# qianduoduolr/FGVC

Measured on AMD Instinct MI355X. Metric: frames/sec + ms/corr-volume, 480p 8-frame clip, 1/2/4/8 MI355X, higher is better.
Workload: dtype f16 + fp6 (e2m3) MFMA operands, f32 accumulate; top-k near-ties re-scored in f64 from f32 features

## Files before the change

### fgvc_amd/csrc/capi.hip

```cpp
#include <stdarg.h>
#include <string.h>

#include "common.hpp"

namespace fgvc {

static thread_local char g_err[512] = "";

void set_error(const char* fmt, ...) {
  va_list ap;
  va_start(ap, fmt);
  vsnprintf(g_err, sizeof(g_err), fmt, ap);
  va_end(ap);
}

int pair_topk_launch(const float*, const float*, const int32_t*, int, int, int, int, int, int, int, int, int, int,
                     const uint8_t*, int32_t*, float*, hipStream_t);
int merge_topk_launch(const int32_t*, const float*, const int32_t*, int, int, int, int, int, float, int, int32_t*,
                      float*, float*, hipStream_t);
int normalize_launch(const float*, float*, int, int, int, int, int, hipStream_t);
int propagate_launch(const float*, const int32_t*, int, const int32_t*, const float*, int, int, int, int, int, int,
                     int, float*, hipStream_t);
int bn_act_launch(const float*, const float*, const float*, const float*, const float*, const float*, float, int, float*,
                  int, int, int, hipStream_t);
int gaussian_launch(const float*, int, int, int, int, float, float*, hipStream_t);
int softargmax_launch(const float*, int, int, int, int, int, int, const float*, float, double*, float*, hipStream_t);
int softargmax_bands();
int corr_volume_f32_launch(const float*, const float*, int, int, int, float, float*, hipStream_t);
int split_bf16_launch(const float*, uint16_t*, long long, int, hipStream_t);
int corr_volume_bf16_launch(const uint16_t*, const uint16_t*, int, int, int, float, float*, int, hipStream_t);
int local_merge_launch(const int32_t*, const float*, int, int, int, int, int, float, int32_t*, float*, float*,
                       hipStream_t);
int local_merge_plan_launch(const int32_t*, const float*, const int32_t*, int, int, int, int, int, int, int, float, int32_t*, float*,
                            float*, hipStream_t);
int topk_coord_launch(const int32_t*, const float*, int, int, int, int, int, float*, hipStream_t);
int topk_coord_rows_launch(const int32_t*, const float*, int, int, int, int, int, int, float*, hipStream_t);
int cycle_chase_launch(const float*, const float*, const float*, int, int, int, int, int, float*, float*, hipStream_t);
int flow_from_lists_launch(const int32_t*, const float*, int, int, int, int, int, int, int, int, int, int, int, float*, uint8_t*, hipStream_t);
int flow_consistency_launch(const float*, const float*, int, int, int, int, float, float*, float*, hipStream_t);
int warp_launch(const float*, const float*, int, int, int, int, int, int, float*, hipStream_t);
int frames_rgb8_to_lab_launch(const uint8_t*, int, int, int, long long, long long, long long, long long, int, int, int, int, int, int, float*,
                              hipStream_t);
int jf_counts_launch(const uint8_t*, const uint8_t*, int, int, int, int, int, int64_t*, hipStream_t);
int jf_tile_rows();
int render_frames_launch(const uint8_t*, long long, long long, uint8_t*, long long, long long, int, int, int, const uint8_t*, long long, long long,
                         const uint8_t*, int, int, const double*, long long, long long, const uint8_t*, long long, long long, const uint8_t*, int,
                         int, const double*, hipStream_t);
void render_tile(int*, int*);
int c2f_refine_launch(const int32_t*, const float*, const float*, const float*, int, int, int, int, int, int, int,
                      int, float, int, float*, int32_t*, float*, hipStream_t);

int conv_split_launch(const uint16_t*, const uint16_t*, const float*, const float*, uint16_t*, float*, int, int, int, int, int,
                      int, int, int, int, int, int, int, int, int*, hipStream_t, unsigned char* y_bank = nullptr, int bank_normalize = 1, const uint16_t* x2 = nullptr,
                      const uint16_t* w2 = nullptr, int Cin2 = 0, int bank_row_bytes = 1024);
int conv_s2_launch(const uint16_t*, const uint16_t*, const float*, uint16_t*, float*, int, int, int, int, int, int, int, int, int,
                   int, int, int, int, int*, const uint16_t*, const float*, float*, int, hipStream_t);
int conv64_launch(const uint16_t*, const uint16_t*, const float*, const float*, const uint16_t*, uint16_t*, float*, int, int, int, int, int, int,
                  int, int, int, int, int*, hipStream_t);
int stem7_launch(const float*, const uint16_t*, const float*, uint16_t*, float*, int, int, int, int, int, int, int, int, int, int, int*,
                 hipStream_t);
int nchw_to_split_nhwc_launch(const float*, uint16_t*, float*, int, int, int, int, int, int, hipStream_t);
int normalize_nhwc_launch(const float*, float*, uint16_t*, int, int, int, int, int, int, hipStream_t);
int nhwc_to_split_launch(float*, uint16_t*, int, int, int, int, int, int, int, hipStream_t);

void set_conv_cot_cap(int);
void set_conv_narrow(int);
void set_conv64_variant(int);
int conv64_probe_read(long long*);
void set_conv_debug(int);
void set_corr6_skew(int);
void set_corr6_sdma(int);
void set_pair_debug(int);
void set_readout_prune(int);
void set_conv_s2_debug(int);
int split_f16x2_launch(const float*, uint16_t*, long long, int, hipStream_t);
int split_f16f6p_launch(const float*, unsigned char*, long long, int, hipStream_t);
int pair_topk_v7_launch(const uint16_t*, const uint16_t*, const int32_t*, int, int, int, int, int, int, int, int, int, const int32_t*, int,
                        int32_t*, float*, int, hipStream_t);
int pair_topk_v5_launch(const uint16_t*, const uint16_t*, const int32_t*, int, int, int, int, int, int, int, int, int, int, const int32_t*,
                        int, int32_t*, float*, hipStream_t);
// ... 41 lines not shown
               "fgvc_set_option: %s = %d switches a profiling ablation on (bits %d: results would be wrong); this library is built without them -- "
               "use libfgvc_hip_ablations.so (FGVC_HIP_LIB)", name, value, ablation_bits(name, value));
#endif
  if (strcmp(name, "corr_debug") == 0) {
    set_corr_debug(value);
    return FGVC_OK;
  }
  if (strcmp(name, "corr8_debug") == 0) {
    set_corr8_debug(value);
    return FGVC_OK;
  }
  if (strcmp(name, "corr6_debug") == 0) {
    set_corr6_debug(value);
    return FGVC_OK;
  }
  if (strcmp(name, "pair_debug") == 0) {
    set_pair_debug(value);
    return FGVC_OK;
  }
  if (strcmp(name, "corr6_sdma") == 0) {
    set_corr6_sdma(value);
    return FGVC_OK;
  }
  if (strcmp(name, "corr6_skew") == 0) {
    set_corr6_skew(value);
    return FGVC_OK;
  }
  if (strcmp(name, "conv_debug") == 0) {
    set_conv_debug(value);
    return FGVC_OK;
  }
  if (strcmp(name, "conv64_variant") == 0) {
    set_conv64_variant(value);
    return FGVC_OK;
  }
  if (strcmp(name, "conv_narrow") == 0) {
    set_conv_narrow(value);
    return FGVC_OK;
  }
  if (strcmp(name, "conv_cot_cap") == 0) {
    FGVC_REQUIRE(value == 0 || value == 64 || value == 128, FGVC_ERR_INVALID_ARG, "fgvc_set_option: conv_cot_cap must be 0, 64 or 128");
    set_conv_cot_cap(value);
    return FGVC_OK;
  }
  if (strcmp(name, "pair_f16_debug") == 0) {
    set_pair_v5_debug(value);
    return FGVC_OK;
  }
  if (strcmp(name, "conv_s2_debug") == 0) {
    set_conv_s2_debug(value);
    return FGVC_OK;
  }
  if (strcmp(name, "readout_prune") == 0) {
    set_readout_prune(value != 0);
    return FGVC_OK;
  }
  set_error("fgvc_set_option: unknown option '%s'", name);
  return FGVC_ERR_INVALID_ARG;
}

int fgvc_r2max_for_radius(float radius) {
  if (!(radius > 0.f)) return -1;
  long long d2 = (long long)ceil((double)radius * (double)radius) + 2;
  if (d2 > FGVC_NO_LIMIT) return FGVC_NO_LIMIT;
  while (d2 >= 0 && !(sqrtf((float)d2) < radius)) --d2;
  return (int)d2;
}

int fgvc_normalize_chw_to_hwc_f32(const float* in, float* out, int n, int C, int HW, int normalize, int c_out,
                                  void* stream) {
  FGVC_REQUIRE(in && out, FGVC_ERR_INVALID_ARG, "fgvc_normalize_chw_to_hwc_f32: null pointer");
  FGVC_REQUIRE(n >= 0 && C > 0 && HW > 0, FGVC_ERR_INVALID_ARG, "fgvc_normalize_chw_to_hwc_f32: bad shape n=%d C=%d HW=%d", n, C, HW);
  FGVC_REQUIRE(C <= 1024, FGVC_ERR_UNSUPPORTED, "fgvc_normalize_chw_to_hwc_f32: C=%d > 1024 (LDS tile)", C);
  FGVC_REQUIRE(n <= 65535, FGVC_ERR_UNSUPPORTED, "fgvc_normalize_chw_to_hwc_f32: n=%d > 65535 frames per call", n);
  FGVC_REQUIRE(c_out >= C, FGVC_ERR_INVALID_ARG, "fgvc_normalize_chw_to_hwc_f32: c_out=%d < C=%d", c_out, C);
  if (n == 0) return FGVC_OK;
  return normalize_launch(in, out, n, C, HW, normalize, c_out, (hipStream_t)stream);
}

int fgvc_pair_topk_f32(const float* qfeat, const float* kfeat, const int32_t* pairs, int n_pairs, int C, int Hq,
                       int Wq, int Hk, int Wk, int r2max, int ry, int rx, int topk, const uint8_t* dense_mask,
                       int32_t* idx_out, float* score_out, void* stream) {
  FGVC_REQUIRE(qfeat && kfeat && pairs && idx_out && score_out, FGVC_ERR_INVALID_ARG, "fgvc_pair_topk_f32: null pointer");
  FGVC_REQUIRE(aligned16(qfeat) && aligned16(kfeat) && aligned16(pairs), FGVC_ERR_INVALID_ARG,
               "fgvc_pair_topk_f32: qfeat/kfeat/pairs must be 16-byte aligned");
  FGVC_REQUIRE(Hq > 0 && Wq > 0 && Hk > 0 && Wk > 0 && n_pairs >= 0, FGVC_ERR_INVALID_ARG,
               "fgvc_pair_topk_f32: bad shape Hq=%d Wq=%d Hk=%d Wk=%d n_pairs=%d", Hq, Wq, Hk, Wk, n_pairs);
  FGVC_REQUIRE(topk >= 1 && topk <= 16, FGVC_ERR_UNSUPPORTED, "fgvc_pair_topk_f32: topk=%d outside 1..16", topk);
  FGVC_REQUIRE(r2max >= 0 && ry >= 0 && rx >= 0, FGVC_ERR_INVALID_ARG, "fgvc_pair_topk_f32: negative mask parameter");
  FGVC_REQUIRE(n_pairs <= 65535, FGVC_ERR_UNSUPPORTED, "fgvc_pair_topk_f32: n_pairs=%d > 65535 per call", n_pairs);
  const bool any_limit = r2max < FGVC_NO_LIMIT || ry < FGVC_NO_LIMIT || rx < FGVC_NO_LIMIT;
  FGVC_REQUIRE(!any_limit || (Hq == Hk && Wq == Wk), FGVC_ERR_INVALID_ARG,
               "fgvc_pair_topk_f32: a spatial mask needs equal query/key grids (local_attention.py:331)");
  FGVC_REQUIRE((long long)Hk * Wk < (1ll << 30) && (long long)Hq * Wq < (1ll << 30), FGVC_ERR_UNSUPPORTED,
               "fgvc_pair_topk_f32: grid too large");
  if (n_pairs == 0) return FGVC_OK;
  FGVC_REQUIRE(dense_mask == nullptr || !any_limit, FGVC_ERR_INVALID_ARG,
               "fgvc_pair_topk_f32: give either the analytic predicate or a dense mask, not both");
  return pair_topk_launch(qfeat, kfeat, pairs, n_pairs, C, Hq, Wq, Hk, Wk, r2max, ry, rx, topk, dense_mask, idx_out,
                          score_out, (hipStream_t)stream);
}

int fgvc_split_f16x2(const float* feat, uint16_t* h_l, int64_t n_pixels, int C, void* stream) {
  FGVC_REQUIRE(feat && h_l, FGVC_ERR_INVALID_ARG, "fgvc_split_f16x2: null pointer");
  FGVC_REQUIRE(n_pixels >= 0 && C > 0 && C % 4 == 0, FGVC_ERR_INVALID_ARG, "fgvc_split_f16x2: C must be a multiple of 4");
  FGVC_REQUIRE(aligned16(feat) && aligned16(h_l), FGVC_ERR_INVALID_ARG, "fgvc_split_f16x2: 16-byte alignment required");
  if (n_pixels == 0) return FGVC_OK;
// ... 687 lines not shown
  FGVC_REQUIRE(x && out, FGVC_ERR_INVALID_ARG, "fgvc_nhwc_to_split_f32: null pointer");
  FGVC_REQUIRE(N >= 0 && C > 0 && C % 32 == 0 && H > 0 && W > 0, FGVC_ERR_INVALID_ARG,
               "fgvc_nhwc_to_split_f32: bad shape (C must be a multiple of 32)");
  FGVC_REQUIRE(conv_pad_ok(H, W, Hp, Wp), FGVC_ERR_INVALID_ARG, "fgvc_nhwc_to_split_f32: padded size %dx%d too small for %dx%d", Hp, Wp, H, W);
  FGVC_REQUIRE(aligned16(x) && aligned16(out), FGVC_ERR_INVALID_ARG, "fgvc_nhwc_to_split_f32: 16-byte alignment required");
  FGVC_REQUIRE((long long)N * H * W * C / 4 < (1ll << 31) * 256, FGVC_ERR_UNSUPPORTED, "fgvc_nhwc_to_split_f32: tensor too large");
  if (N == 0) return FGVC_OK;
  return nhwc_to_split_launch(x, out, N, C, H, W, Hp, Wp, relu, (hipStream_t)stream);
}

static int normalize_split_common(const char* what, const float* in, float* out_f32, uint16_t* out_split, int N, int C, int H, int W,
                                  int normalize, int fmt, void* stream) {
  FGVC_REQUIRE(in && (out_f32 || out_split), FGVC_ERR_INVALID_ARG, "%s: null pointer", what);
  FGVC_REQUIRE(N >= 0 && C > 0 && C % 4 == 0 && H > 0 && W > 0, FGVC_ERR_INVALID_ARG, "%s: bad shape", what);
  FGVC_REQUIRE(aligned16(in) && aligned16(out_f32) && aligned16(out_split), FGVC_ERR_INVALID_ARG, "%s: 16-byte alignment required", what);
  if (N == 0) return FGVC_OK;
  return normalize_nhwc_launch(in, out_f32, out_split, N, C, H, W, normalize, fmt, (hipStream_t)stream);
}

int fgvc_normalize_split_nhwc_f32(const float* in, float* out_f32, uint16_t* out_split, int N, int C, int H, int W, int normalize,
                                  void* stream) {
  return normalize_split_common("fgvc_normalize_split_nhwc_f32", in, out_f32, out_split, N, C, H, W, normalize, 0, stream);
}

int fgvc_normalize_split_f16x2_nhwc_f32(const float* in, float* out_f32, uint16_t* out_split, int N, int C, int H, int W,
                                        int normalize, void* stream) {
  return normalize_split_common("fgvc_normalize_split_f16x2_nhwc_f32", in, out_f32, out_split, N, C, H, W, normalize, 1, stream);
}

int fgvc_normalize_split_f16f6p_nhwc_f32(const float* in, uint8_t* rows, int N, int C, int H, int W, int normalize, void* stream) {
  FGVC_REQUIRE(C == 256, FGVC_ERR_UNSUPPORTED, "fgvc_normalize_split_f16f6p_nhwc_f32: C=%d unsupported (256 only)", C);
  return normalize_split_common("fgvc_normalize_split_f16f6p_nhwc_f32", in, nullptr, reinterpret_cast<uint16_t*>(rows), N, C, H, W, normalize, 2, stream);
}

int fgvc_normalize_split_f16f6x_nhwc_f32(const float* in, uint8_t* rows, int N, int C, int H, int W, int normalize, void* stream) {
  FGVC_REQUIRE(C == 256, FGVC_ERR_UNSUPPORTED, "fgvc_normalize_split_f16f6x_nhwc_f32: C=%d unsupported (256 only)", C);
  return normalize_split_common("fgvc_normalize_split_f16f6x_nhwc_f32", in, nullptr, reinterpret_cast<uint16_t*>(rows), N, C, H, W, normalize, 3, stream);
}

int fgvc_normalize_nhwc_f32(const float* in, float* out, int N, int C, int H, int W, int normalize, void* stream) {
  FGVC_REQUIRE(in && out, FGVC_ERR_INVALID_ARG, "fgvc_normalize_nhwc_f32: null pointer");
  return fgvc_normalize_split_nhwc_f32(in, out, nullptr, N, C, H, W, normalize, stream);
}

int fgvc_gaussian_labels_f32(const float* points, int P, int Hf, int Wf, int stride, float sigma, float* out,
                             void* stream) {
  FGVC_REQUIRE(points && out, FGVC_ERR_INVALID_ARG, "fgvc_gaussian_labels_f32: null pointer");
  FGVC_REQUIRE(P > 0 && Hf > 0 && Wf > 0 && stride >= 1 && sigma > 0.f, FGVC_ERR_INVALID_ARG, "fgvc_gaussian_labels_f32: bad shape");
  return gaussian_launch(points, P, Hf, Wf, stride, sigma, out, (hipStream_t)stream);
}

size_t fgvc_softargmax_workspace_bytes(int n_frames, int P) {
  if (n_frames < 0 || P < 0) return 0;
  return (size_t)n_frames * P * (softargmax_bands() * (2 * 5 + 1) + 1) * sizeof(float);
}

int fgvc_softargmax_top5_f32(const float* labels, int n_frames, int Hf, int Wf, int P, int h, int w,
                             const float* gauss_points, float sigma, double* coords, void* workspace, void* stream) {
  FGVC_REQUIRE(labels && coords, FGVC_ERR_INVALID_ARG, "fgvc_softargmax_top5_f32: null pointer");
  FGVC_REQUIRE(n_frames >= 0 && Hf > 0 && Wf > 0 && P > 0 && h > 0 && w > 0, FGVC_ERR_INVALID_ARG, "fgvc_softargmax_top5_f32: bad shape");
  FGVC_REQUIRE((long long)h * w < (1ll << 31) && h * w >= 5, FGVC_ERR_UNSUPPORTED, "fgvc_softargmax_top5_f32: h*w out of range");
  FGVC_REQUIRE(n_frames <= 65535 && sigma > 0.f, FGVC_ERR_INVALID_ARG, "fgvc_softargmax_top5_f32: bad n_frames/sigma");
  FGVC_REQUIRE(workspace != nullptr || n_frames == 0, FGVC_ERR_INVALID_ARG,
               "fgvc_softargmax_top5_f32: workspace of fgvc_softargmax_workspace_bytes() bytes required");
  FGVC_REQUIRE(P <= 65535, FGVC_ERR_UNSUPPORTED, "fgvc_softargmax_top5_f32: P > 65535");
  if (n_frames == 0) return FGVC_OK;
  return softargmax_launch(labels, n_frames, Hf, Wf, P, h, w, gauss_points, sigma, coords,
                           static_cast<float*>(workspace), (hipStream_t)stream);
}

}
```

### fgvc_amd/csrc/post.hip

```cpp
#include "common.hpp"

namespace fgvc {

__global__ __launch_bounds__(256) void normalize_chw_to_hwc_kernel(const float* __restrict__ in,
                                                                     float* __restrict__ out, int C, int HW,
                                                                     int normalize, int Cout) {
  extern __shared__ float tile[];
  float* part = tile + (size_t)C * 33;
  float* inv = part + 8 * 32;
  const int tid = threadIdx.x;
  const int px = tid & 31, grp = tid >> 5;
  const int p0 = blockIdx.x * 32;
  const size_t frame = blockIdx.y;
  const float* src = in + frame * (size_t)C * HW;
  float ss = 0.f;
  const int p = p0 + px;
  for (int c = grp; c < C; c += 8) {
    const float v = (p < HW) ? src[(size_t)c * HW + p] : 0.f;
    tile[c * 33 + px] = v;
    ss = fmaf(v, v, ss);
  }
  part[grp * 32 + px] = ss;
  __syncthreads();
  if (tid < 32) {
// ... 402 lines not shown
            if (slot < RO_CELLS) cells[slot] = c;
          }
        }
      }
      __syncthreads();
      const int nc = n_cells;
      if (nc > RO_CELLS) {
        if (tid == 0) need_scan[map] = 1;
        return;
      }
      for (int k = tid >> 2; k < nc; k += RO_BLOCK / 4) {
        const int c = cells[k];
        const int i = c / Wf, j = c - i * Wf;
        const int ya = first_fine_of_cell(i, sy, Hf, h), yb = (i + 1 >= Hf) ? h : first_fine_of_cell(i + 1, sy, Hf, h);
        const int xa = first_fine_of_cell(j, sx, Wf, w), xb = (j + 1 >= Wf) ? w : first_fine_of_cell(j + 1, sx, Wf, w);
        for (int y = ya + (tid & 3); y < yb; y += 4)
          for (int x = xa; x < xb; ++x) {
            const float v = fine_value(lab, Hf, Wf, P, sy, sx, y, x);
            if (v >= tau) {
              const int slot = atomicAdd(&n_cand, 1);
              if (slot < RO_CAND) { cand_v[slot] = v; cand_i[slot] = y * w + x; }
            }
          }
      }
      __syncthreads();
      if (n_cand > RO_CAND || n_cand < K) {
        if (tid == 0) need_scan[map] = 1;
        return;
      }
    }
  }
  if (map_max > 0.f) {
    const int n = n_cand;
    for (int t = tid; t < n; t += RO_BLOCK) {
      const float v = cand_v[t];
      const int id = cand_i[t];
      int rank = 0;
      for (int u = 0; u < n; ++u) {
        const float vu = cand_v[u];
        rank += (vu > v || (vu == v && cand_i[u] > id)) ? 1 : 0;
      }
      if (rank < K) {
        part_v[o * K + rank] = v;
        part_i[o * K + rank] = id;
      }
    }
  }
  if (tid == 0) {
    part_sum[o] = map_max > 0.f ? 1.f : 0.f;
    need_scan[map] = 0;
  }
}

__global__ __launch_bounds__(64) void softargmax_merge_kernel(const float* __restrict__ part_v,
                                                               const int* __restrict__ part_i,
                                                               const float* __restrict__ part_sum, int nbands, int w,
                                                               int n_maps, double* __restrict__ coords) {
  constexpr int K = RO_K;
  const int m = blockIdx.x * 64 + threadIdx.x;
  if (m >= n_maps) return;
  TopKHi<K> top;
  top.init();
  float sum = 0.f;
  for (int b = 0; b < nbands; ++b) {
    const size_t o = (size_t)m * nbands + b;
    sum += part_sum[o];
    for (int j = 0; j < K; ++j) {
      const int id = part_i[o * K + j];
      const float v = part_v[o * K + j];
      if (id >= 0 && top.accepts(v, id)) top.insert(v, id);
    }
  }
  double* o = coords + (size_t)m * 2;
  if (sum == 0.f) {
    o[0] = -1.0;
    o[1] = -1.0;
    return;
  }
  float tot = 0.f;
#pragma unroll
  for (int j = K - 1; j >= 0; --j) tot += top.v[j];
  tot += 1e-9f;
  double ax = 0.0, ay = 0.0;
#pragma unroll
  for (int j = K - 1; j >= 0; --j) {
    const float wgt = top.v[j] / tot;
    ax += (double)(top.ix[j] % w) * (double)wgt;
    ay += (double)(top.ix[j] / w) * (double)wgt;
  }
  o[0] = ax;
  o[1] = ay;
}

template <bool VEC>
__global__ __launch_bounds__(256) void bn_act_kernel(const float* __restrict__ x, const float* __restrict__ res,
                                                      const float* __restrict__ mean, const float* __restrict__ var,
                                                      const float* __restrict__ gamma, const float* __restrict__ beta,
                                                      float eps, int relu, float* __restrict__ out, int C, int HW,
                                                      long long n) {
  const long long stride = (long long)gridDim.x * 256;
  if constexpr (VEC) {
    const long long n4 = n >> 2;
    const int HW4 = HW >> 2;
    for (long long i = (long long)blockIdx.x * 256 + threadIdx.x; i < n4; i += stride) {
      const int c = (int)((i / HW4) % C);
      const float inv = 1.0f / sqrtf(var[c] + eps);
// ... 20 lines not shown
    }
  }
}

int bn_act_launch(const float* x, const float* res, const float* mean, const float* var, const float* gamma,
                  const float* beta, float eps, int relu, float* out, int N, int C, int HW, hipStream_t s) {
  const long long n = (long long)N * C * HW;
  const bool vec = (HW % 4 == 0) && ((reinterpret_cast<uintptr_t>(x) | reinterpret_cast<uintptr_t>(out) |
                                      reinterpret_cast<uintptr_t>(res)) & 15u) == 0;
  const long long work = vec ? n / 4 : n;
  const int grid = (int)((work + 255) / 256 < 256 * 16 ? (work + 255) / 256 : 256 * 16);
  if (vec)
    bn_act_kernel<true><<<grid, 256, 0, s>>>(x, res, mean, var, gamma, beta, eps, relu, out, C, HW, n);
  else
    bn_act_kernel<false><<<grid, 256, 0, s>>>(x, res, mean, var, gamma, beta, eps, relu, out, C, HW, n);
  FGVC_CHECK_LAUNCH("fgvc_bn_act_f32");
  return FGVC_OK;
}

int normalize_launch(const float* in, float* out, int n, int C, int HW, int normalize, int Cout, hipStream_t s) {
  dim3 grid(cdiv(HW, 32), n);
  const size_t lds = ((size_t)C * 33 + 8 * 32 + 32) * sizeof(float);
  if (lds > 48 * 1024) {
    hipError_t e = hipFuncSetAttribute(reinterpret_cast<const void*>(normalize_chw_to_hwc_kernel),
                                       hipFuncAttributeMaxDynamicSharedMemorySize, (int)lds);
    if (e != hipSuccess) {
      set_error("fgvc_normalize_chw_to_hwc_f32: cannot reserve %zu B of LDS: %s", lds, hipGetErrorString(e));
      return FGVC_ERR_LAUNCH;
    }
  }
  normalize_chw_to_hwc_kernel<<<grid, 256, lds, s>>>(in, out, C, HW, normalize, Cout);
  FGVC_CHECK_LAUNCH("fgvc_normalize_chw_to_hwc_f32");
  return FGVC_OK;
}

int propagate_launch(const float* labels, const int32_t* slot_frame, int T, const int32_t* idx, const float* weight,
                     int Hq, int Wq, int Hk, int Wk, int P, int topk, int window_L, float* out, hipStream_t s) {
  const long long n = (long long)Hq * Wq * P;
  propagate_kernel<<<(unsigned)((n + 255) / 256), 256, 0, s>>>(labels, slot_frame, T, idx, weight, Hq, Wq, Hk, Wk, P,
                                                               topk, window_L, out);
  FGVC_CHECK_LAUNCH("fgvc_propagate_topk_f32");
  return FGVC_OK;
}

int gaussian_launch(const float* points, int P, int Hf, int Wf, int stride, float sigma, float* out, hipStream_t s) {
  const long long n = (long long)Hf * Wf * P;
  gaussian_labels_kernel<<<(unsigned)((n + 255) / 256), 256, 0, s>>>(points, P, Hf, Wf, stride,
                                                                     2.f * sigma * sigma, out);
  FGVC_CHECK_LAUNCH("fgvc_gaussian_labels_f32");
  return FGVC_OK;
}

int softargmax_bands() { return 8; }
static int g_readout_prune = 1;
void set_readout_prune(int v) { g_readout_prune = v; }

int softargmax_launch(const float* labels, int n_frames, int Hf, int Wf, int P, int h, int w,
                      const float* gauss_points, float sigma, double* coords, float* ws, hipStream_t s) {
  const int nb = softargmax_bands();
  const size_t maps = (size_t)n_frames * P;
  float* part_v = ws;
  int* part_i = reinterpret_cast<int*>(ws + maps * nb * RO_K);
  float* part_sum = ws + 2 * maps * nb * RO_K;
  int* need_scan = reinterpret_cast<int*>(ws + maps * nb * (2 * RO_K + 1));
  if (g_readout_prune) {
    softargmax_pruned_kernel<<<dim3(P, n_frames), RO_BLOCK, 0, s>>>(labels, Hf, Wf, P, h, w, nb, gauss_points,
                                                                2.f * sigma * sigma, part_v, part_i, part_sum, need_scan);
  }
  dim3 grid(P, n_frames, nb);
  softargmax_band_kernel<<<grid, 256, 0, s>>>(labels, Hf, Wf, P, h, w, nb, gauss_points, 2.f * sigma * sigma, part_v,
                                              part_i, part_sum, g_readout_prune ? need_scan : nullptr);
  softargmax_merge_kernel<<<cdiv((int)maps, 64), 64, 0, s>>>(part_v, part_i, part_sum, nb, w, (int)maps, coords);
  FGVC_CHECK_LAUNCH("fgvc_softargmax_top5_f32");
  return FGVC_OK;
}

}
```

### fgvc_amd/ops.py

```python
from __future__ import annotations

import ctypes as C
import functools
import math
from dataclasses import dataclass
from typing import Optional, Tuple

import torch

from . import _lib
from ._lib import NO_LIMIT, PAIR_MASKED, WEIGHT_COSINE, WEIGHT_RAW, WEIGHT_SOFTMAX


@dataclass(frozen=True)
class MaskSpec:
    r2max: int = NO_LIMIT
    ry: int = NO_LIMIT
    rx: int = NO_LIMIT

    @property
    def is_none(self) -> bool:
        return self.r2max >= NO_LIMIT and self.ry >= NO_LIMIT and self.rx >= NO_LIMIT

    @staticmethod
# ... 986 lines not shown
    x = _chk(x, torch.float32, "x")
    N, H, W, C = x.shape
    shape, dt = ((N, H * W, 4 if fmt == "f16f6x" else 2, C), torch.int16) if split else ((N, H * W, C), torch.float32)
    if out is None:
        out = torch.empty(shape, device=x.device, dtype=dt)
    else:
        assert tuple(out.shape) == shape and out.dtype == dt and out.is_contiguous() and out.device == x.device
    if fmt in ("f16f6", "f16f6x"):
        assert C == 256
        _lib.call(f"fgvc_normalize_split_{fmt}p_nhwc_f32" if fmt == "f16f6" else "fgvc_normalize_split_f16f6x_nhwc_f32", _ptr(x), _ptr(out), N, C, H, W,
                  int(normalize), _stream(x))
        return out
    _lib.call("fgvc_normalize_split_f16x2_nhwc_f32" if fmt == "f16" else "fgvc_normalize_split_nhwc_f32", _ptr(x),
              _ptr(None if split else out), _ptr(out if split else None), N, C, H, W, int(normalize), _stream(x))
    return out


def unsplit_f16x2(split: torch.Tensor) -> torch.Tensor:
    v = split.view(torch.float16).float()
    return (v[..., 0, :] + v[..., 1, :]) * (1.0 / 16384.0)


def unsplit_act(split: torch.Tensor, fmt: int, scale_log2: int = 0) -> torch.Tensor:
    n5 = split.shape
    if fmt == ACT_BF16X2:
        v = split.view(torch.bfloat16).float()
        return (v[..., :32] + v[..., 32:]).reshape(*n5[:3], -1)
    b = split.contiguous().view(torch.uint8).reshape(*n5[:4], 128)
    h = b[..., :64].contiguous().view(torch.float16).float()
    if fmt == ACT_F16X2:
        l = b[..., 64:].contiguous().view(torch.float16).float()
    elif fmt == ACT_F16F6:
        l = _e2m3_decode(torch.cat([b[..., 64:80], b[..., 96:104]], dim=-1), b[..., 104])
    else:
        l = b[..., 64:96].contiguous().view(torch.float8_e4m3fn).float() * 2.0 ** -F8_BX
    return ((h + l) * 2.0 ** -scale_log2).reshape(*n5[:3], -1)


def unsplit_bf16(split: torch.Tensor) -> torch.Tensor:
    v = split.view(torch.bfloat16).float()
    return v[..., 0, :] + v[..., 1, :]


def gaussian_labels(points: torch.Tensor, Hf: int, Wf: int, stride: int, sigma: float = 6.0,
                    out: Optional[torch.Tensor] = None) -> torch.Tensor:
    points = _chk(points.to(torch.float32), torch.float32, "points")
    P = points.shape[0]
    if out is None:
        out = torch.empty((Hf * Wf, P), device=points.device, dtype=torch.float32)
    _lib.call("fgvc_gaussian_labels_f32", _ptr(points), P, Hf, Wf, stride, float(sigma), _ptr(out), _stream(points))
    return out


def softargmax_top5(labels: torch.Tensor, Hf: int, Wf: int, h: int, w: int,
                    gauss_points: Optional[torch.Tensor] = None, sigma: float = 6.0) -> torch.Tensor:
    labels = _chk(labels, torch.float32, "labels")
    n, P = labels.shape[0], labels.shape[2]
    assert labels.shape[1] == Hf * Wf
    if gauss_points is not None:
        gauss_points = _chk(gauss_points.to(torch.float32), torch.float32, "gauss_points")
        assert gauss_points.shape == (P, 2)
    coords = torch.empty((n, P, 2), device=labels.device, dtype=torch.float64)
    ws_bytes = _lib.load().fgvc_softargmax_workspace_bytes(n, P)
    ws = torch.empty((max(ws_bytes, 4) + 3) // 4, device=labels.device, dtype=torch.float32)
    _lib.call("fgvc_softargmax_top5_f32", _ptr(labels), n, Hf, Wf, P, h, w, _ptr(gauss_points), float(sigma),
              _ptr(coords), _ptr(ws), _stream(labels))
    return coords



def pil_nearest_index(n_in: int, n_out: int) -> torch.Tensor:
    a, xo, out = n_in / n_out, n_in / n_out * 0.5, []
    for _ in range(n_out):
        out.append(min(int(xo), n_in - 1))
        xo += a
    return torch.tensor(out, dtype=torch.int64)


def seg_max_label(seg_map: torch.Tensor, Hf: int, Wf: int, out: Optional[torch.Tensor] = None) -> torch.Tensor:
    seg_map = _chk(seg_map, torch.uint8, "seg_map")
    hp, wp = seg_map.shape
    if out is None:
        out = torch.empty((1,), device=seg_map.device, dtype=torch.int32)
    _lib.call("fgvc_seg_max_label_u8", _ptr(seg_map), hp, wp, Hf, Wf, _ptr(out), _stream(seg_map))
    return out


def seg_onehot_labels(seg_map: torch.Tensor, Hf: int, Wf: int, C: int, out: Optional[torch.Tensor] = None) -> torch.Tensor:
    seg_map = _chk(seg_map, torch.uint8, "seg_map")
    hp, wp = seg_map.shape
    if out is None:
        out = torch.empty((Hf * Wf, C), device=seg_map.device, dtype=torch.float32)
    else:
        assert out.is_contiguous() and out.shape == (Hf * Wf, C) and out.dtype == torch.float32
    _lib.call("fgvc_seg_onehot_labels_u8", _ptr(seg_map), hp, wp, Hf, Wf, C, _ptr(out), _stream(seg_map))
    return out


def seg_hard_onehot(labels: torch.Tensor, out: Optional[torch.Tensor] = None) -> torch.Tensor:
    labels = _chk(labels, torch.float32, "labels")
    C = labels.shape[-1]
    if out is None:
        out = torch.empty_like(labels)
    else:
        assert out.is_contiguous() and out.shape == labels.shape and out.dtype == torch.float32
    _lib.call("fgvc_seg_hard_onehot_f32", _ptr(labels), labels.numel() // C, C, _ptr(out), _stream(labels))
    return out


def seg_readout(labels: torch.Tensor, Hf: int, Wf: int, pad_shape: Tuple[int, int], pad: Tuple[int, int, int, int],
                out_shape: Tuple[int, int], norm: bool = True, out: Optional[torch.Tensor] = None) -> torch.Tensor:
    labels = _chk(labels, torch.float32, "labels")
    n, C = labels.shape[0], labels.shape[2]
    assert labels.shape[1] == Hf * Wf
    (hp, wp), (lw, uw, lh, uh), (h0, w0) = pad_shape, pad, out_shape
    if out is None:
        out = torch.empty((n, h0, w0), device=labels.device, dtype=torch.uint8)
# ... 241 lines not shown
```

Before: 2060.

## Replace softargmax prune with chunk-stats, threshold, candidate-cell multi-kernel pipeline

Adds a new default readout pruning path built from four kernels. The first gathers per-chunk max, argmax and min over coarse label cells. The second finds a top-5 threshold tau from fine windows around the peak cells. The third collects coarse cells whose 2x2 neighbourhood bound can reach tau, and the fourth scans only those cells at fine resolution. This replaces a per-map pruned kernel, aiming to cut fine-resolution work and spread the coarse scan across many more blocks. The cost is extra launches, a larger workspace, and fallback to a full scan when the candidate count overflows RO_CELLS; the old path stays available as mode 2.

```diff
diff --git a/fgvc_amd/csrc/capi.hip b/fgvc_amd/csrc/capi.hip
--- a/fgvc_amd/csrc/capi.hip
+++ b/fgvc_amd/csrc/capi.hip
@@ -26,6 +26,7 @@
 int gaussian_launch(const float*, int, int, int, int, float, float*, hipStream_t);
 int softargmax_launch(const float*, int, int, int, int, int, int, const float*, float, double*, float*, hipStream_t);
 int softargmax_bands();
+size_t softargmax_workspace_words_per_map();
 int corr_volume_f32_launch(const float*, const float*, int, int, int, float, float*, hipStream_t);
 int split_bf16_launch(const float*, uint16_t*, long long, int, hipStream_t);
 int corr_volume_bf16_launch(const uint16_t*, const uint16_t*, int, int, int, float, float*, int, hipStream_t);
@@ -173,7 +174,8 @@
     return FGVC_OK;
   }
   if (strcmp(name, "readout_prune") == 0) {
-    set_readout_prune(value != 0);
+    FGVC_REQUIRE(value >= 0 && value <= 2, FGVC_ERR_INVALID_ARG, "fgvc_set_option: readout_prune must be 0, 1 or 2");
+    set_readout_prune(value);
     return FGVC_OK;
   }
   set_error("fgvc_set_option: unknown option '%s'", name);
@@ -967,7 +969,7 @@
 
 size_t fgvc_softargmax_workspace_bytes(int n_frames, int P) {
   if (n_frames < 0 || P < 0) return 0;
-  return (size_t)n_frames * P * (softargmax_bands() * (2 * 5 + 1) + 1) * sizeof(float);
+  return (size_t)n_frames * P * softargmax_workspace_words_per_map() * sizeof(float);
 }
 
 int fgvc_softargmax_top5_f32(const float* labels, int n_frames, int Hf, int Wf, int P, int h, int w,
diff --git a/fgvc_amd/csrc/post.hip b/fgvc_amd/csrc/post.hip
--- a/fgvc_amd/csrc/post.hip
+++ b/fgvc_amd/csrc/post.hip
@@ -478,6 +478,386 @@
   }
 }
 
+constexpr int RO_CHUNKS = 64;
+constexpr int RO_MIN_CHUNK = 32;
+constexpr int RO_LT = 16;
+constexpr int RO_T = 256;
+
+__device__ __forceinline__ int block_top5(TopKHi<RO_K>& loc, float (*sh_v)[RO_T / WAVE], int (*sh_i)[RO_T / WAVE], float (&ov)[RO_K],
+                                          int (&oi)[RO_K]) {
+  constexpr int NW = RO_T / WAVE;
+  const int lane = threadIdx.x & (WAVE - 1), wv = threadIdx.x / WAVE;
+  int n = 0;
+#pragma unroll
+  for (int r = 0; r < RO_K; ++r) {
+    float bv = loc.v[0];
+    int bi = loc.ix[0];
+#pragma unroll
+    for (int off = WAVE / 2; off >= 1; off >>= 1) {
+      const float tv = __shfl_xor(bv, off, WAVE);
+      const int ti = __shfl_xor(bi, off, WAVE);
+      const bool b = tv > bv || (tv == bv && ti > bi);
+      bv = b ? tv : bv;
+      bi = b ? ti : bi;
+    }
+    if (lane == 0) { sh_v[r][wv] = bv; sh_i[r][wv] = bi; }
+    __syncthreads();
+    bv = sh_v[r][0];
+    bi = sh_i[r][0];
+#pragma unroll
+    for (int k = 1; k < NW; ++k) {
+      const float tv = sh_v[r][k];
+      const int ti = sh_i[r][k];
+      const bool b = tv > bv || (tv == bv && ti > bi);
+      bv = b ? tv : bv;
+      bi = b ? ti : bi;
+    }
+    ov[r] = bv;
+    oi[r] = bi;
+    n += bi >= 0 ? 1 : 0;
+    const bool pop = bi >= 0 && bi == loc.ix[0];
+#pragma unroll
+    for (int j = 0; j < RO_K - 1; ++j) {
+      loc.v[j] = pop ? loc.v[j + 1] : loc.v[j];
+      loc.ix[j] = pop ? loc.ix[j + 1] : loc.ix[j];
+    }
+    loc.v[RO_K - 1] = pop ? -INFINITY : loc.v[RO_K - 1];
+    loc.ix[RO_K - 1] = pop ? -1 : loc.ix[RO_K - 1];
+  }
+  return n;
+}
+
+template <bool VEC>
+__device__ __forceinline__ void load_labels(const float* __restrict__ px, int np, float (&v)[RO_LT]) {
+  if constexpr (VEC) {
+#pragma unroll
+    for (int q = 0; q < RO_LT / 4; ++q) {
+      f32x4 t = {0.f, 0.f, 0.f, 0.f};
+      if (4 * q < np) t = reinterpret_cast<const f32x4*>(px)[q];
+      v[4 * q] = t.x; v[4 * q + 1] = t.y; v[4 * q + 2] = t.z; v[4 * q + 3] = t.w;
+    }
+  } else {
+#pragma unroll
+    for (int j = 0; j < RO_LT; ++j) v[j] = j < np ? px[j] : 0.f;
+  }
+}
+
+template <bool VEC>
+__global__ __launch_bounds__(RO_T) void softargmax_stats_kernel(const float* __restrict__ labels, int n_coarse, int P, int chunk_len,
+                                                                int skip_frame0, float* __restrict__ stats) {
+  constexpr int NW = RO_T / WAVE;
+  __shared__ float sh_mx[NW][RO_LT];
+  __shared__ int sh_am[NW][RO_LT];
+  __shared__ float sh_mn[NW][RO_LT];
+  const int tid = threadIdx.x;
+  const int chunk = blockIdx.x, f = blockIdx.y, p0 = blockIdx.z * RO_LT;
+  if (skip_frame0 && f == 0) return;
+  const int np = imin(RO_LT, P - p0);
+  const float* lab = labels + (size_t)f * n_coarse * P + p0;
+  const int c_lo = chunk * chunk_len, c_hi = imin(n_coarse, c_lo + chunk_len);
+  float mx[RO_LT], mn[RO_LT];
+  int am[RO_LT];
+#pragma unroll
+  for (int j = 0; j < RO_LT; ++j) { mx[j] = -INFINITY; mn[j] = INFINITY; am[j] = c_lo; }
+  for (int c = c_lo + tid; c < c_hi; c += RO_T) {
+    float v[RO_LT];
+    load_labels<VEC>(lab + (size_t)c * P, np, v);
+#pragma unroll
+    for (int j = 0; j < RO_LT; ++j) {
+      if (v[j] > mx[j]) { mx[j] = v[j]; am[j] = c; }
+      mn[j] = (v[j] < mn[j] || v[j] != v[j]) ? v[j] : mn[j];
+    }
+  }
+#pragma unroll
+  for (int j = 0; j < RO_LT; ++j) {
+#pragma unroll
+    for (int off = WAVE / 2; off >= 1; off >>= 1) {
+      const float ov = __shfl_xor(mx[j], off, WAVE), on = __shfl_xor(mn[j], off, WAVE);
+      const int oa = __shfl_xor(am[j], off, WAVE);
+      const bool b = ov > mx[j] || (ov == mx[j] && oa < am[j]);
+      mx[j] = b ? ov : mx[j];
+      am[j] = b ? oa : am[j];
+      mn[j] = (mn[j] != mn[j]) ? mn[j] : ((on < mn[j] || on != on) ? on : mn[j]);
+    }
+  }
+  if ((tid & (WAVE - 1)) == 0) {
+#pragma unroll
+    for (int j = 0; j < RO_LT; ++j) { sh_mx[tid / WAVE][j] = mx[j]; sh_am[tid / WAVE][j] = am[j]; sh_mn[tid / WAVE][j] = mn[j]; }
+  }
+  __syncthreads();
+  if (tid < np) {
+    float m = sh_mx[0][tid], n = sh_mn[0][tid];
+    int a = sh_am[0][tid];
+    for (int k = 1; k < NW; ++k) {
+      const float ov = sh_mx[k][tid], on = sh_mn[k][tid];
+      const int oa = sh_am[k][tid];
+      if (ov > m || (ov == m && oa < a)) { m = ov; a = oa; }
+      n = (n != n) ? n : ((on < n || on != on) ? on : n);
+    }
+    float* o = stats + (((size_t)f * RO_CHUNKS + chunk) * P + p0 + tid) * 3;
+    o[0] = m;
+    o[1] = __int_as_float(a);
+    o[2] = n;
+  }
+}
+
+__global__ __launch_bounds__(RO_T) void softargmax_tau_kernel(const float* __restrict__ labels, int Hf, int Wf, int P, int h, int w,
+                                                              int nbands, int n_chunks, const float* __restrict__ gauss_points,
+                                                              float two_sigma2, const float* __restrict__ stats,
+                                                              float* __restrict__ part_v, int* __restrict__ part_i,
+                                                              float* __restrict__ part_sum, int* __restrict__ need_scan,
+                                                              float* __restrict__ tau_ws, int* __restrict__ n_cells) {
+  constexpr int K = RO_K;
+  __shared__ float sh_v[K][RO_T / WAVE];
+  __shared__ int sh_i[K][RO_T / WAVE];
+  __shared__ float peak_v[K];
+  __shared__ int peak_c[K];
+  __shared__ float min_s;
+  __shared__ int win[K][4];
+  __shared__ int win_off[K + 1];
+  const int tid = threadIdx.x;
+  const int pl = blockIdx.x, f = blockIdx.y;
+  const size_t map = (size_t)f * P + pl;
+  const size_t o = map * nbands;
+  const float* lab = labels + (size_t)f * Hf * Wf * P + pl;
+  const float sy = (float)Hf / (float)h, sx = (float)Wf / (float)w;
+  const bool analytic = (gauss_points != nullptr) && f == 0;
+  for (int j = tid; j < nbands * K; j += RO_T) {
+    part_v[o * K + j] = -INFINITY;
+    part_i[o * K + j] = -1;
+  }
+  for (int j = tid; j < nbands; j += RO_T) part_sum[o + j] = 0.f;
+  if (tid == 0) n_cells[map] = 0;
+  float ov[K];
+  int oi[K];
+  if (analytic) {
+    const float cx = gauss_points[2 * pl], cy = gauss_points[2 * pl + 1];
+    const int xc = (int)fminf(fmaxf(rintf(cx), 0.f), (float)(w - 1)), yc = (int)fminf(fmaxf(rintf(cy), 0.f), (float)(h - 1));
+    TopKHi<K> loc;
+    loc.init();
+    if (tid < 169) {
+      const int y = yc + tid / 13 - 6, x = xc + tid % 13 - 6;
+      if (y >= 0 && y < h && x >= 0 && x < w) {
+        const float v = gauss_value(x, y, cx, cy, two_sigma2);
+        if (loc.accepts(v, y * w + x)) loc.insert(v, y * w + x);
+      }
+    }
+    const int n = block_top5(loc, sh_v, sh_i, ov, oi);
+    if (tid == 0) {
+      const bool ok = n == K && ov[0] >= 0.f;
+      if (ok && ov[0] > 0.f) {
+#pragma unroll
+        for (int j = 0; j < K; ++j) { part_v[o * K + j] = ov[j]; part_i[o * K + j] = oi[j]; }
+        part_sum[o] = 1.f;
+      }
+      need_scan[map] = ok ? 0 : 1;
+      tau_ws[map] = NAN;
+    }
+    return;
+  }
+  if (Hf > 2 * h || Wf > 2 * w) {
+    if (tid == 0) { need_scan[map] = 1; tau_ws[map] = NAN; }
+    return;
+  }
+  if (tid < WAVE) {
+    float cm = -INFINITY, cn = INFINITY;
+    int ca = 0;
+    if (tid < n_chunks) {
+      const float* st = stats + (((size_t)f * RO_CHUNKS + tid) * P + pl) * 3;
+      cm = st[0];
+      ca = __float_as_int(st[1]);
+      cn = st[2];
+    }
+#pragma unroll
+    for (int off = WAVE / 2; off >= 1; off >>= 1) {
+      const float on = __shfl_xor(cn, off, WAVE);
+      cn = (cn != cn) ? cn : ((on < cn || on != on) ? on : cn);
+    }
+    if (tid == 0) min_s = cn;
+    int id = tid < n_chunks ? (WAVE - 1 - tid) : -1;
+#pragma unroll
+    for (int r = 0; r < K; ++r) {
+      float bv = cm;
+      int bi = id, ba = ca;
+#pragma unroll
+      for (int off = WAVE / 2; off >= 1; off >>= 1) {
+        const float tv = __shfl_xor(bv, off, WAVE);
+        const int ti = __shfl_xor(bi, off, WAVE), ta = __shfl_xor(ba, off, WAVE);
+        const bool b = ti >= 0 && (bi < 0 || tv > bv || (tv == bv && ti > bi));
+        bv = b ? tv : bv;
+        bi = b ? ti : bi;
+        ba = b ? ta : ba;
+      }
+      if (tid == 0) { peak_v[r] = bi >= 0 ? bv : -INFINITY; peak_c[r] = bi >= 0 ? ba : -1; }
+      if (bi >= 0 && bi == id) id = -1;
+    }
+  }
+  __syncthreads();
+  const float map_max = peak_v[0];
+  if (!(min_s >= 0.f) || !(map_max < INFINITY)) {
+    if (tid == 0) { need_scan[map] = 1; tau_ws[map] = NAN; }
+    return;
+  }
+  if (!(map_max > 0.f)) {
+    if (tid == 0) { need_scan[map] = 0; tau_ws[map] = NAN; }
+    return;
+  }
+  if (tid < K) {
+    int y_lo = 0, y_hi = 0, x_lo = 0, x_hi = 0;
+    const int cell0 = peak_c[tid];
+    if (cell0 >= 0) {
+      const int ci = cell0 / Wf, cj = cell0 - ci * Wf;
+      y_lo = first_fine_of_cell(imax(ci - 1, 0), sy, Hf, h);
+      y_hi = first_fine_of_cell(imin(ci + 2, Hf), sy, Hf, h);
+      x_lo = first_fine_of_cell(imax(cj - 1, 0), sx, Wf, w);
+      x_hi = first_fine_of_cell(imin(cj + 2, Wf), sx, Wf, w);
+      if (ci + 2 >= Hf) y_hi = h;
+      if (cj + 2 >= Wf) x_hi = w;
+      y_hi = imin(y_hi, y_lo + 32);
+      x_hi = imin(x_hi, x_lo + 32);
+    }
+    win[tid][0] = y_lo; win[tid][1] = y_hi; win[tid][2] = x_lo; win[tid][3] = x_hi;
+  }
+  __syncthreads();
+  if (tid == 0) {
+    int acc = 0;
+    for (int r = 0; r < K; ++r) {
+      win_off[r] = acc;
+      acc += (win[r][1] - win[r][0]) * (win[r][3] - win[r][2]);
+    }
+    win_off[K] = acc;
+  }
+  __syncthreads();
+  TopKHi<K> loc;
+  loc.init();
+  const int nn = win_off[K];
+  for (int t = tid; t < nn; t += RO_T) {
+    int r = 0;
+#pragma unroll
+    for (int q = 1; q < K; ++q) r += t >= win_off[q] ? 1 : 0;
+    const int nx = win[r][3] - win[r][2], u = t - win_off[r];
+    const int y = win[r][0] + u / nx, x = win[r][2] + u % nx;
+    bool seen = false;
+    for (int q = 0; q < r; ++q) seen |= y >= win[q][0] && y < win[q][1] && x >= win[q][2] && x < win[q][3];
+    if (!seen) {
+      const float v = fine_value(lab, Hf, Wf, P, sy, sx, y, x);
+      if (loc.accepts(v, t)) loc.insert(v, t);
+    }
+  }
+  const int n = block_top5(loc, sh_v, sh_i, ov, oi);
+  if (tid == 0) {
+    if (n < K) {
+      need_scan[map] = 1;
+      tau_ws[map] = NAN;
+    } else {
+      tau_ws[map] = ov[K - 1];
+    }
+  }
+}
+
+template <bool VEC>
+__global__ __launch_bounds__(RO_T) void softargmax_cells_kernel(const float* __restrict__ labels, int Hf, int Wf, int P,
+                                                                const float* __restrict__ tau_ws, int* __restrict__ n_cells,
+                                                                int* __restrict__ cells) {
+  __shared__ int cnt[RO_LT];
+  __shared__ int base[RO_LT];
+  __shared__ int lst[RO_LT][RO_T];
+  const int tid = threadIdx.x;
+  const int f = blockIdx.y, p0 = blockIdx.z * RO_LT;
+  const int np = imin(RO_LT, P - p0);
+  const int n_coarse = Hf * Wf;
+  const size_t map0 = (size_t)f * P + p0;
+  float tau[RO_LT];
+  bool any = false;
+#pragma unroll
+  for (int j = 0; j < RO_LT; ++j) {
+    tau[j] = j < np ? tau_ws[map0 + j] : NAN;
+    any |= tau[j] == tau[j];
+  }
+  if (!any) return;
+  if (tid < RO_LT) cnt[tid] = 0;
+  __syncthreads();
+  const int c = blockIdx.x * RO_T + tid;
+  if (c < n_coarse) {
+    const float* lab = labels + (size_t)f * n_coarse * P + p0;
+    const int i = c / Wf, j0 = c - i * Wf;
+    const int i1 = i + (i < Hf - 1 ? 1 : 0), j1 = j0 + (j0 < Wf - 1 ? 1 : 0);
+    float a[RO_LT], b[RO_LT], d[RO_LT], e[RO_LT];
+    load_labels<VEC>(lab + ((size_t)i * Wf + j0) * P, np, a);
+    load_labels<VEC>(lab + ((size_t)i * Wf + j1) * P, np, b);
+    load_labels<VEC>(lab + ((size_t)i1 * Wf + j0) * P, np, d);
+    load_labels<VEC>(lab + ((size_t)i1 * Wf + j1) * P, np, e);
+#pragma unroll
+    for (int j = 0; j < RO_LT; ++j) {
+      const float B = fmaxf(fmaxf(a[j], b[j]), fmaxf(d[j], e[j]));
+      if (B * (1.f + 4e-6f) >= tau[j]) {
+        const int slot = atomicAdd(&cnt[j], 1);
+        lst[j][slot] = c;
+      }
+    }
+  }
+  __syncthreads();
+  if (tid < np && cnt[tid] > 0) base[tid] = atomicAdd(&n_cells[map0 + tid], cnt[tid]);
+  __syncthreads();
+  for (int j = 0; j < np; ++j) {
+    const int n = cnt[j];
+    if (n == 0) continue;
+    const int b0 = base[j];
+    for (int k = tid; k < n; k += RO_T)
+      if (b0 + k < RO_CELLS) cells[(map0 + j) * RO_CELLS + b0 + k] = lst[j][k];
+  }
+}
+
+__global__ __launch_bounds__(RO_T) void softargmax_finish_kernel(const float* __restrict__ labels, int Hf, int Wf, int P, int h, int w,
+                                                                 int nbands, const float* __restrict__ tau_ws,
+                                                                 const int* __restrict__ n_cells, const int* __restrict__ cells,
+                                                                 float* __restrict__ part_v, int* __restrict__ part_i,
+                                                                 float* __restrict__ part_sum, int* __restrict__ need_scan) {
+  constexpr int K = RO_K;
+  __shared__ float sh_v[K][RO_T / WAVE];
+  __shared__ int sh_i[K][RO_T / WAVE];
+  const int tid = threadIdx.x;
+  const int pl = blockIdx.x, f = blockIdx.y;
+  const size_t map = (size_t)f * P + pl;
+  const size_t o = map * nbands;
+  const float tau = tau_ws[map];
+  if (!(tau == tau)) return;
+  const int nc = n_cells[map];
+  if (nc > RO_CELLS) {
+    if (tid == 0) need_scan[map] = 1;
+    return;
+  }
+  const float* lab = labels + (size_t)f * Hf * Wf * P + pl;
+  const float sy = (float)Hf / (float)h, sx = (float)Wf / (float)w;
+  TopKHi<K> loc;
+  loc.init();
+  const int sub = tid & 15, ry = sub >> 2, rx = sub & 3;
+  for (int k = tid >> 4; k < nc; k += RO_T / 16) {
+    const int c = cells[map * RO_CELLS + k];
+    const int i = c / Wf, j = c - i * Wf;
+    const int ya = first_fine_of_cell(i, sy, Hf, h), yb = (i + 1 >= Hf) ? h : first_fine_of_cell(i + 1, sy, Hf, h);
+    const int xa = first_fine_of_cell(j, sx, Wf, w), xb = (j + 1 >= Wf) ? w : first_fine_of_cell(j + 1, sx, Wf, w);
+    for (int y = ya + ry; y < yb; y += 4)
+      for (int x = xa + rx; x < xb; x += 4) {
+        const float v = fine_value(lab, Hf, Wf, P, sy, sx, y, x);
+        if (v >= tau && loc.accepts(v, y * w + x)) loc.insert(v, y * w + x);
+      }
+  }
+  float ov[K];
+  int oi[K];
+  const int n = block_top5(loc, sh_v, sh_i, ov, oi);
+  if (tid == 0) {
+    if (n < K) {
+      need_scan[map] = 1;
+    } else {
+#pragma unroll
+      for (int j = 0; j < K; ++j) { part_v[o * K + j] = ov[j]; part_i[o * K + j] = oi[j]; }
+      part_sum[o] = 1.f;
+      need_scan[map] = 0;
+    }
+  }
+}
+
 __global__ __launch_bounds__(64) void softargmax_merge_kernel(const float* __restrict__ part_v,
                                                                const int* __restrict__ part_i,
                                                                const float* __restrict__ part_sum, int nbands, int w,
@@ -604,6 +984,7 @@
 }
 
 int softargmax_bands() { return 8; }
+size_t softargmax_workspace_words_per_map() { return (size_t)softargmax_bands() * (2 * RO_K + 1) + 3 + 3 * RO_CHUNKS + RO_CELLS; }
 static int g_readout_prune = 1;
 void set_readout_prune(int v) { g_readout_prune = v; }
 
@@ -615,7 +996,30 @@
   int* part_i = reinterpret_cast<int*>(ws + maps * nb * RO_K);
   float* part_sum = ws + 2 * maps * nb * RO_K;
   int* need_scan = reinterpret_cast<int*>(ws + maps * nb * (2 * RO_K + 1));
-  if (g_readout_prune) {
+  float* tau = reinterpret_cast<float*>(need_scan + maps);
+  int* n_cells = reinterpret_cast<int*>(tau + maps);
+  float* stats = reinterpret_cast<float*>(n_cells + maps);
+  int* cells = reinterpret_cast<int*>(stats + maps * 3 * RO_CHUNKS);
+  if (g_readout_prune == 1) {
+    const int n_coarse = Hf * Wf;
+    const int chunk_len = imax(cdiv(n_coarse, RO_CHUNKS), RO_MIN_CHUNK), n_chunks = cdiv(n_coarse, chunk_len);
+    const int tiles = cdiv(P, RO_LT);
+    const bool vec = (P % 4 == 0) && (reinterpret_cast<uintptr_t>(labels) & 15u) == 0;
+    const bool prunable = !(Hf > 2 * h || Wf > 2 * w);
+    const int skip0 = gauss_points != nullptr ? 1 : 0;
+    if (prunable) {
+      if (vec) softargmax_stats_kernel<true><<<dim3(n_chunks, n_frames, tiles), RO_T, 0, s>>>(labels, n_coarse, P, chunk_len, skip0, stats);
+      else softargmax_stats_kernel<false><<<dim3(n_chunks, n_frames, tiles), RO_T, 0, s>>>(labels, n_coarse, P, chunk_len, skip0, stats);
+    }
+    softargmax_tau_kernel<<<dim3(P, n_frames), RO_T, 0, s>>>(labels, Hf, Wf, P, h, w, nb, n_chunks, gauss_points, 2.f * sigma * sigma,
+                                                             stats, part_v, part_i, part_sum, need_scan, tau, n_cells);
+    if (prunable) {
+      if (vec) softargmax_cells_kernel<true><<<dim3(cdiv(n_coarse, RO_T), n_frames, tiles), RO_T, 0, s>>>(labels, Hf, Wf, P, tau, n_cells, cells);
+      else softargmax_cells_kernel<false><<<dim3(cdiv(n_coarse, RO_T), n_frames, tiles), RO_T, 0, s>>>(labels, Hf, Wf, P, tau, n_cells, cells);
+      softargmax_finish_kernel<<<dim3(P, n_frames), RO_T, 0, s>>>(labels, Hf, Wf, P, h, w, nb, tau, n_cells, cells, part_v, part_i,
+                                                                  part_sum, need_scan);
+    }
+  } else if (g_readout_prune == 2) {
     softargmax_pruned_kernel<<<dim3(P, n_frames), RO_BLOCK, 0, s>>>(labels, Hf, Wf, P, h, w, nb, gauss_points,
                                                                 2.f * sigma * sigma, part_v, part_i, part_sum, need_scan);
   }
diff --git a/fgvc_amd/ops.py b/fgvc_amd/ops.py
--- a/fgvc_amd/ops.py
+++ b/fgvc_amd/ops.py
@@ -1062,8 +1062,19 @@
     return out
 
 
+def softargmax_workspace(n_frames: int, P: int, device) -> torch.Tensor:
+    ws_bytes = _lib.load().fgvc_softargmax_workspace_bytes(n_frames, P)
+    return torch.empty((max(ws_bytes, 4) + 3) // 4, device=device, dtype=torch.int32)
+
+
+def softargmax_need_scan(workspace: torch.Tensor, n_frames: int, P: int) -> torch.Tensor:
+    maps = n_frames * P
+    return workspace[maps * 8 * 11:maps * 8 * 11 + maps].view(n_frames, P)
+
+
 def softargmax_top5(labels: torch.Tensor, Hf: int, Wf: int, h: int, w: int,
-                    gauss_points: Optional[torch.Tensor] = None, sigma: float = 6.0) -> torch.Tensor:
+                    gauss_points: Optional[torch.Tensor] = None, sigma: float = 6.0,
+                    workspace: Optional[torch.Tensor] = None) -> torch.Tensor:
     labels = _chk(labels, torch.float32, "labels")
     n, P = labels.shape[0], labels.shape[2]
     assert labels.shape[1] == Hf * Wf
@@ -1071,8 +1082,8 @@
         gauss_points = _chk(gauss_points.to(torch.float32), torch.float32, "gauss_points")
         assert gauss_points.shape == (P, 2)
     coords = torch.empty((n, P, 2), device=labels.device, dtype=torch.float64)
-    ws_bytes = _lib.load().fgvc_softargmax_workspace_bytes(n, P)
-    ws = torch.empty((max(ws_bytes, 4) + 3) // 4, device=labels.device, dtype=torch.float32)
+    ws = softargmax_workspace(n, P, labels.device) if workspace is None else workspace
+    assert ws.is_contiguous() and ws.numel() * ws.element_size() >= _lib.load().fgvc_softargmax_workspace_bytes(n, P)
     _lib.call("fgvc_softargmax_top5_f32", _ptr(labels), n, Hf, Wf, P, h, w, _ptr(gauss_points), float(sigma),
               _ptr(coords), _ptr(ws), _stream(labels))
     return coords
```

Result: no change. 2069, median of 6 (+0.4%).
